# DCMMC/halo2-scaffold

Measured on NVIDIA B200. Metric: bn254_g1_msm_points_per_s, higher is better.
Workload: dtype u32 limbs (254-bit modular integers)

## Files before the change

halo2_scaffold_b200/csrc/ec.cuh:

```cuda
#pragma once
#include "field.cuh"

namespace h2b {

struct Affine {
    Fq x, y;
};
struct XYZZ {
    Fq x, y, zz, zzz;
};

__device__ __forceinline__ bool affine_is_identity(const Affine& p) { return fp_is_zero(p.x) && fp_is_zero(p.y); }
__device__ __forceinline__ bool xyzz_is_identity(const XYZZ& p) { return fp_is_zero(p.zz); }
__device__ __forceinline__ XYZZ xyzz_identity() {
    XYZZ r;
    r.x = fp_zero<FQ>(); r.y = fp_zero<FQ>(); r.zz = fp_zero<FQ>(); r.zzz = fp_zero<FQ>();
    return r;
}
__device__ __forceinline__ Affine affine_load(const void* p) {
    Affine a;
    a.x = fp_load<FQ>(p);
    a.y = fp_load<FQ>(reinterpret_cast<const uint4*>(p) + 2);
    return a;
}
// ... 65 lines not shown
    Affine q = q_in;
    if (neg) q.y = fp_neg(q.y);
    if (xyzz_is_identity(acc)) {
        acc.x = q.x; acc.y = q.y; acc.zz = fp_one<FQ>(); acc.zzz = fp_one<FQ>();
        return;
    }
    Fq u2 = fp_mul(q.x, acc.zz);
    Fq s2 = fp_mul(q.y, acc.zzz);
    Fq p = fp_sub(u2, acc.x);
    Fq r = fp_sub(s2, acc.y);
    if (fp_is_zero(p)) {
        if (fp_is_zero(r)) acc = xyzz_double_affine(q);
        else acc = xyzz_identity();
        return;
    }
    Fq pp = fp_sqr(p);
    Fq ppp = fp_mul(p, pp);
    Fq qq = fp_mul(acc.x, pp);
    Fq x3 = fp_sub(fp_sub(fp_sqr(r), ppp), fp_dbl(qq));
#ifdef H2B_MADD_MUL2
    Fq y3 = fp_mul2(r, fp_sub(qq, x3), fp_neg(acc.y), ppp);
#else
    Fq y3 = fp_sub(fp_mul(r, fp_sub(qq, x3)), fp_mul(acc.y, ppp));
#endif
    acc.x = x3;
    acc.y = y3;
    acc.zz = fp_mul(acc.zz, pp);
    acc.zzz = fp_mul(acc.zzz, ppp);
}

__device__ __forceinline__ void xyzz_add_affine_lazy(XYZZ& acc, const Affine& q_in, bool neg) {
    if (affine_is_identity(q_in)) return;
    Affine q = q_in;
    if (neg) q.y = fp_neg(q.y);
    if (xyzz_is_identity(acc)) {
        acc.x = q.x; acc.y = q.y; acc.zz = fp_one<FQ>(); acc.zzz = fp_one<FQ>();
        return;
    }
    Fq u2 = fp_mul_lazy(q.x, acc.zz);
    Fq s2 = fp_mul_lazy(q.y, acc.zzz);
    Fq p = fp_sub_lazy(u2, acc.x);
    Fq r = fp_sub_lazy(s2, acc.y);
    if (fp_is_zero_lazy(p)) {
        if (fp_is_zero_lazy(r)) acc = xyzz_double_affine(q);
        else acc = xyzz_identity();
        return;
    }
    Fq pp = fp_sqr_lazy(p);
    Fq ppp = fp_mul_lazy(p, pp);
    Fq qq = fp_mul_lazy(acc.x, pp);
    Fq yppp = fp_mul_lazy(acc.y, ppp);
    Fq x3 = fp_sub_lazy(fp_sub_lazy(fp_sqr_lazy(r), ppp), fp_add_lazy(qq, qq));
    Fq y3 = fp_sub_lazy(fp_mul_lazy(r, fp_sub_lazy(qq, x3)), yppp);
    acc.x = x3;
    acc.y = y3;
    acc.zz = fp_mul_lazy(acc.zz, pp);
    acc.zzz = fp_mul_lazy(acc.zzz, ppp);
}
__device__ __forceinline__ XYZZ xyzz_canon(const XYZZ& a) {
    XYZZ r;
    r.x = fp_canon(a.x); r.y = fp_canon(a.y); r.zz = fp_canon(a.zz); r.zzz = fp_canon(a.zzz);
    return r;
}

template <bool SHARED> __device__ __forceinline__ void xyzz_add_body(XYZZ& acc, const XYZZ& b);
static __device__ __noinline__ XYZZ xyzz_add_shared(XYZZ acc, XYZZ b) {
    xyzz_add_body<true>(acc, b);
    return acc;
}
template <bool SHARED = false>
__device__ __forceinline__ void xyzz_add(XYZZ& acc, const XYZZ& b) {
    if (SHARED) acc = xyzz_add_shared(acc, b);
    else xyzz_add_body<false>(acc, b);
}
template <bool SHARED>
__device__ __forceinline__ void xyzz_add_body(XYZZ& acc, const XYZZ& b) {
    if (xyzz_is_identity(b)) return;
    if (xyzz_is_identity(acc)) { acc = b; return; }
    Fq u1 = fq_m<SHARED>(acc.x, b.zz);
    Fq u2 = fq_m<SHARED>(b.x, acc.zz);
    Fq s1 = fq_m<SHARED>(acc.y, b.zzz);
    Fq s2 = fq_m<SHARED>(b.y, acc.zzz);
    Fq p = fp_sub(u2, u1);
    Fq r = fp_sub(s2, s1);
    if (fp_is_zero(p)) {
// ... 76 lines not shown
```

halo2_scaffold_b200/csrc/field.cuh:

```cuda
#pragma once
#include <cstdint>

#ifdef H2B_EMU
#include "cuda_emu.h"
#else
#include <cuda_runtime.h>
#define H2B_LAUNCH(kern, grid, block, smem, stream, ...) \
    (h2b::count_launch(), kern<<<(grid), (block), (smem), (stream)>>>(__VA_ARGS__))
#define H2B_DYN_SMEM(T, name)                                   \
    extern __shared__ __align__(16) unsigned char _h2b_dsm[];   \
    T* name = reinterpret_cast<T*>(_h2b_dsm)
#include "field_asm.inc"
#endif

namespace h2b {

extern unsigned long long g_launch_count;
inline void count_launch() { __atomic_fetch_add(&g_launch_count, 1ull, __ATOMIC_RELAXED); }

enum FieldId { FR = 0, FQ = 1 };

template <int F> struct FpParams;
template <> struct FpParams<FR> {
    __host__ __device__ static constexpr uint32_t P(int i) {
// ... 101 lines not shown
    Fp<F> r;
    if (F == FR) fr_sub_asm(r.l, a.l, b.l); else fq_sub_asm(r.l, a.l, b.l);
    return r;
}
template <int F> __device__ __forceinline__ Fp<F> fp_mul_lazy(const Fp<F>& a, const Fp<F>& b) {
    Fp<F> r;
    if (F == FR) fr_mul_lazy_asm(r.l, a.l, b.l); else fq_mul_lazy_asm(r.l, a.l, b.l);
    return r;
}
template <int F> __device__ __forceinline__ Fp<F> fp_sqr_lazy(const Fp<F>& a) {
#ifdef H2B_SQR_AS_MUL
    return fp_mul_lazy(a, a);
#else
    Fp<F> r;
    if (F == FR) fr_sqr_lazy_asm(r.l, a.l); else fq_sqr_lazy_asm(r.l, a.l);
    return r;
#endif
}
template <int F> __device__ __forceinline__ Fp<F> fp_add_lazy(const Fp<F>& a, const Fp<F>& b) {
    Fp<F> r;
    if (F == FR) fr_add_lazy_asm(r.l, a.l, b.l); else fq_add_lazy_asm(r.l, a.l, b.l);
    return r;
}
template <int F> __device__ __forceinline__ Fp<F> fp_sub_lazy(const Fp<F>& a, const Fp<F>& b) {
    Fp<F> r;
    if (F == FR) fr_sub_lazy_asm(r.l, a.l, b.l); else fq_sub_lazy_asm(r.l, a.l, b.l);
    return r;
}
template <int F> __device__ __forceinline__ Fp<F> fp_canon(const Fp<F>& a) {
    Fp<F> r;
    if (F == FR) fr_canon_asm(r.l, a.l); else fq_canon_asm(r.l, a.l);
    return r;
}
#else
template <int F> inline bool fp_geq_p(const uint32_t* t) {
    for (int i = 7; i >= 0; --i) {
        if (t[i] > FpParams<F>::P(i)) return true;
        if (t[i] < FpParams<F>::P(i)) return false;
    }
    return true;
}
template <int F> inline void fp_sub_p(uint32_t* t) {
    int64_t bw = 0;
    for (int i = 0; i < 8; ++i) {
        int64_t d = (int64_t)t[i] - FpParams<F>::P(i) + bw;
        t[i] = (uint32_t)d;
        bw = d >> 32;
    }
}
template <int F> inline void fp_mont_emu(const Fp<F>& a, const Fp<F>& b, uint32_t (&t)[10]) {
    for (int i = 0; i < 8; ++i) {
        uint64_t c = 0;
        for (int j = 0; j < 8; ++j) { c += (uint64_t)a.l[j] * b.l[i] + t[j]; t[j] = (uint32_t)c; c >>= 32; }
        c += t[8]; t[8] = (uint32_t)c; t[9] = (uint32_t)(c >> 32);
        uint32_t m = t[0] * FpParams<F>::INV;
        c = (uint64_t)m * FpParams<F>::P(0) + t[0]; c >>= 32;
        for (int j = 1; j < 8; ++j) { c += (uint64_t)m * FpParams<F>::P(j) + t[j]; t[j - 1] = (uint32_t)c; c >>= 32; }
        c += t[8]; t[7] = (uint32_t)c; t[8] = t[9] + (uint32_t)(c >> 32);
    }
}
template <int F> inline Fp<F> fp_mul(const Fp<F>& a, const Fp<F>& b) {
    uint32_t t[10] = {0};
    fp_mont_emu(a, b, t);
    Fp<F> r;
    if (t[8] || fp_geq_p<F>(t)) fp_sub_p<F>(t);
    for (int i = 0; i < 8; ++i) r.l[i] = t[i];
// ... 18 lines not shown
}
template <int F> inline void fp_2p(uint32_t (&q)[8]) {
    uint64_t c = 0;
    for (int i = 0; i < 8; ++i) { c += 2 * (uint64_t)FpParams<F>::P(i); q[i] = (uint32_t)c; c >>= 32; }
}
template <int F> inline Fp<F> fp_mul_lazy(const Fp<F>& a, const Fp<F>& b) {
    uint32_t t[10] = {0};
    fp_mont_emu(a, b, t);
    Fp<F> r; for (int i = 0; i < 8; ++i) r.l[i] = t[i];
    return r;
}
template <int F> inline Fp<F> fp_sqr_lazy(const Fp<F>& a) { return fp_mul_lazy(a, a); }
template <int F> inline Fp<F> fp_add_lazy(const Fp<F>& a, const Fp<F>& b) {
    uint32_t q[8], t[8], s[8]; fp_2p<F>(q);
    uint64_t c = 0; int64_t bw = 0;
    for (int i = 0; i < 8; ++i) { c += (uint64_t)a.l[i] + b.l[i]; t[i] = (uint32_t)c; c >>= 32; }
    for (int i = 0; i < 8; ++i) { int64_t d = (int64_t)t[i] - q[i] + bw; s[i] = (uint32_t)d; bw = d >> 32; }
    Fp<F> r; for (int i = 0; i < 8; ++i) r.l[i] = bw ? t[i] : s[i];
    return r;
}
template <int F> inline Fp<F> fp_sub_lazy(const Fp<F>& a, const Fp<F>& b) {
    uint32_t q[8], t[8]; fp_2p<F>(q);
    int64_t bw = 0;
    for (int i = 0; i < 8; ++i) { int64_t d = (int64_t)a.l[i] - b.l[i] + bw; t[i] = (uint32_t)d; bw = d >> 32; }
    if (bw) { uint64_t c = 0; for (int i = 0; i < 8; ++i) { c += (uint64_t)t[i] + q[i]; t[i] = (uint32_t)c; c >>= 32; } }
    Fp<F> r; for (int i = 0; i < 8; ++i) r.l[i] = t[i];
    return r;
}
template <int F> inline Fp<F> fp_canon(const Fp<F>& a) {
    Fp<F> r = a;
    if (fp_geq_p<F>(r.l)) fp_sub_p<F>(r.l);
    return r;
}
#endif

template <int F> __device__ __forceinline__ bool fp_is_zero_lazy(const Fp<F>& a) {
    uint32_t o = 0, d = 0;
#pragma unroll
    for (int i = 0; i < 8; ++i) { o |= a.l[i]; d |= a.l[i] ^ FpParams<F>::P(i); }
    return o == 0 || d == 0;
}

template <int F> __device__ __forceinline__ Fp<F> fp_neg(const Fp<F>& a) { return fp_sub(fp_zero<F>(), a); }
template <int F> __device__ __forceinline__ Fp<F> fp_dbl(const Fp<F>& a) { return fp_add(a, a); }
template <int F> __device__ __forceinline__ Fp<F> fp_from_mont(const Fp<F>& a) {
    Fp<F> o = fp_zero<F>();
    o.l[0] = 1;
    return fp_mul(a, o);
}
template <int F> __device__ __forceinline__ Fp<F> fp_to_mont(const Fp<F>& a) {
    Fp<F> r2;
#pragma unroll
    for (int i = 0; i < 8; ++i) r2.l[i] = FpParams<F>::R2(i);
    return fp_mul(a, r2);
}
template <int F> __device__ __noinline__ Fp<F> fp_inv(const Fp<F>& a) {
    Fp<F> r = fp_one<F>();
#pragma unroll
    for (int w = 7; w >= 0; --w) {
        uint32_t word = FpParams<F>::P(w);
        if (w == 0) word -= 2;
#pragma unroll 1
        for (int i = 31; i >= 0; --i) {
            r = fp_sqr(r);
            if ((word >> i) & 1) r = fp_mul(r, a);
        }
// ... 16 lines not shown
```

halo2_scaffold_b200/csrc/field_asm.inc:

```

__device__ __forceinline__ void fr_mul_asm(uint32_t (&r)[8], const uint32_t (&a)[8], const uint32_t (&b)[8]) {
    asm(
        "{\n\t"
        ".reg .u32 e0, e1, e2, e3, e4, e5, e6, e7, o0, o1, o2, o3, o4, o5, o6, o7, m, t0, t1, t2, t3, t4, t5, t6, t7, s0, s1, s2, s3, s4, s5, s6, s7, bw;\n\t"
        ".reg .pred pz;\n\t"
        "mul.lo.u32 o0, %9, %16;\n\t"
        "mul.hi.u32 o1, %9, %16;\n\t"
        "mul.lo.u32 o2, %11, %16;\n\t"
        "mul.hi.u32 o3, %11, %16;\n\t"
        "mul.lo.u32 o4, %13, %16;\n\t"
        "mul.hi.u32 o5, %13, %16;\n\t"
        "mul.lo.u32 o6, %15, %16;\n\t"
        "mul.hi.u32 o7, %15, %16;\n\t"
        "mul.lo.u32 e0, %8, %16;\n\t"
        "mul.hi.u32 e1, %8, %16;\n\t"
        "mul.lo.u32 e2, %10, %16;\n\t"
        "mul.hi.u32 e3, %10, %16;\n\t"
        "mul.lo.u32 e4, %12, %16;\n\t"
        "mul.hi.u32 e5, %12, %16;\n\t"
        "mul.lo.u32 e6, %14, %16;\n\t"
        "mul.hi.u32 e7, %14, %16;\n\t"
        "mul.lo.u32 m, e0, 0xefffffff;\n\t"
        "mad.lo.cc.u32 o0, 0x43e1f593, m, o0;\n\t"
        "madc.hi.cc.u32 o1, 0x43e1f593, m, o1;\n\t"
// ... 1222 lines not shown
        "sub.cc.u32 s0, t0, 0xf0000001;\n\t"
        "subc.cc.u32 s1, t1, 0x43e1f593;\n\t"
        "subc.cc.u32 s2, t2, 0x79b97091;\n\t"
        "subc.cc.u32 s3, t3, 0x2833e848;\n\t"
        "subc.cc.u32 s4, t4, 0x8181585d;\n\t"
        "subc.cc.u32 s5, t5, 0xb85045b6;\n\t"
        "subc.cc.u32 s6, t6, 0xe131a029;\n\t"
        "subc.cc.u32 s7, t7, 0x30644e72;\n\t"
        "subc.u32 bw, 0x00000000, 0x00000000;\n\t"
        "setp.ne.u32 pz, bw, 0;\n\t"
        "selp.u32 %0, t0, s0, pz;\n\t"
        "setp.ne.u32 pz, bw, 0;\n\t"
        "selp.u32 %1, t1, s1, pz;\n\t"
        "setp.ne.u32 pz, bw, 0;\n\t"
        "selp.u32 %2, t2, s2, pz;\n\t"
        "setp.ne.u32 pz, bw, 0;\n\t"
        "selp.u32 %3, t3, s3, pz;\n\t"
        "setp.ne.u32 pz, bw, 0;\n\t"
        "selp.u32 %4, t4, s4, pz;\n\t"
        "setp.ne.u32 pz, bw, 0;\n\t"
        "selp.u32 %5, t5, s5, pz;\n\t"
        "setp.ne.u32 pz, bw, 0;\n\t"
        "selp.u32 %6, t6, s6, pz;\n\t"
        "setp.ne.u32 pz, bw, 0;\n\t"
        "selp.u32 %7, t7, s7, pz;\n\t"
        "}\n\t"
        : "=r"(r[0]), "=r"(r[1]), "=r"(r[2]), "=r"(r[3]), "=r"(r[4]), "=r"(r[5]), "=r"(r[6]), "=r"(r[7])
        : "r"(a[0]), "r"(a[1]), "r"(a[2]), "r"(a[3]), "r"(a[4]), "r"(a[5]), "r"(a[6]), "r"(a[7]), "r"(b[0]), "r"(b[1]), "r"(b[2]), "r"(b[3]), "r"(b[4]), "r"(b[5]), "r"(b[6]), "r"(b[7]));
}

__device__ __forceinline__ void fr_sub_asm(uint32_t (&r)[8], const uint32_t (&a)[8], const uint32_t (&b)[8]) {
    asm(
        "{\n\t"
        ".reg .u32 t0, t1, t2, t3, t4, t5, t6, t7, q0, q1, q2, q3, q4, q5, q6, q7, bw;\n\t"
        ".reg .pred pz;\n\t"
        "sub.cc.u32 t0, %8, %16;\n\t"
        "subc.cc.u32 t1, %9, %17;\n\t"
        "subc.cc.u32 t2, %10, %18;\n\t"
        "subc.cc.u32 t3, %11, %19;\n\t"
        "subc.cc.u32 t4, %12, %20;\n\t"
        "subc.cc.u32 t5, %13, %21;\n\t"
        "subc.cc.u32 t6, %14, %22;\n\t"
        "subc.cc.u32 t7, %15, %23;\n\t"
        "subc.u32 bw, 0x00000000, 0x00000000;\n\t"
        "and.b32 q0, bw, 0xf0000001;\n\t"
        "and.b32 q1, bw, 0x43e1f593;\n\t"
        "and.b32 q2, bw, 0x79b97091;\n\t"
        "and.b32 q3, bw, 0x2833e848;\n\t"
        "and.b32 q4, bw, 0x8181585d;\n\t"
        "and.b32 q5, bw, 0xb85045b6;\n\t"
        "and.b32 q6, bw, 0xe131a029;\n\t"
        "and.b32 q7, bw, 0x30644e72;\n\t"
        "add.cc.u32 %0, t0, q0;\n\t"
        "addc.cc.u32 %1, t1, q1;\n\t"
        "addc.cc.u32 %2, t2, q2;\n\t"
        "addc.cc.u32 %3, t3, q3;\n\t"
        "addc.cc.u32 %4, t4, q4;\n\t"
        "addc.cc.u32 %5, t5, q5;\n\t"
        "addc.cc.u32 %6, t6, q6;\n\t"
        "addc.u32 %7, t7, q7;\n\t"
        "}\n\t"
        : "=r"(r[0]), "=r"(r[1]), "=r"(r[2]), "=r"(r[3]), "=r"(r[4]), "=r"(r[5]), "=r"(r[6]), "=r"(r[7])
        : "r"(a[0]), "r"(a[1]), "r"(a[2]), "r"(a[3]), "r"(a[4]), "r"(a[5]), "r"(a[6]), "r"(a[7]), "r"(b[0]), "r"(b[1]), "r"(b[2]), "r"(b[3]), "r"(b[4]), "r"(b[5]), "r"(b[6]), "r"(b[7]));
}

__device__ __forceinline__ void fq_mul_asm(uint32_t (&r)[8], const uint32_t (&a)[8], const uint32_t (&b)[8]) {
    asm(
// ... 1244 lines not shown
        "sub.cc.u32 s0, t0, 0xd87cfd47;\n\t"
        "subc.cc.u32 s1, t1, 0x3c208c16;\n\t"
        "subc.cc.u32 s2, t2, 0x6871ca8d;\n\t"
        "subc.cc.u32 s3, t3, 0x97816a91;\n\t"
        "subc.cc.u32 s4, t4, 0x8181585d;\n\t"
        "subc.cc.u32 s5, t5, 0xb85045b6;\n\t"
        "subc.cc.u32 s6, t6, 0xe131a029;\n\t"
        "subc.cc.u32 s7, t7, 0x30644e72;\n\t"
        "subc.u32 bw, 0x00000000, 0x00000000;\n\t"
        "setp.ne.u32 pz, bw, 0;\n\t"
        "selp.u32 %0, t0, s0, pz;\n\t"
        "setp.ne.u32 pz, bw, 0;\n\t"
        "selp.u32 %1, t1, s1, pz;\n\t"
        "setp.ne.u32 pz, bw, 0;\n\t"
        "selp.u32 %2, t2, s2, pz;\n\t"
        "setp.ne.u32 pz, bw, 0;\n\t"
        "selp.u32 %3, t3, s3, pz;\n\t"
        "setp.ne.u32 pz, bw, 0;\n\t"
        "selp.u32 %4, t4, s4, pz;\n\t"
        "setp.ne.u32 pz, bw, 0;\n\t"
        "selp.u32 %5, t5, s5, pz;\n\t"
        "setp.ne.u32 pz, bw, 0;\n\t"
        "selp.u32 %6, t6, s6, pz;\n\t"
        "setp.ne.u32 pz, bw, 0;\n\t"
        "selp.u32 %7, t7, s7, pz;\n\t"
        "}\n\t"
        : "=r"(r[0]), "=r"(r[1]), "=r"(r[2]), "=r"(r[3]), "=r"(r[4]), "=r"(r[5]), "=r"(r[6]), "=r"(r[7])
        : "r"(a[0]), "r"(a[1]), "r"(a[2]), "r"(a[3]), "r"(a[4]), "r"(a[5]), "r"(a[6]), "r"(a[7]), "r"(b[0]), "r"(b[1]), "r"(b[2]), "r"(b[3]), "r"(b[4]), "r"(b[5]), "r"(b[6]), "r"(b[7]));
}

__device__ __forceinline__ void fq_sub_asm(uint32_t (&r)[8], const uint32_t (&a)[8], const uint32_t (&b)[8]) {
    asm(
        "{\n\t"
        ".reg .u32 t0, t1, t2, t3, t4, t5, t6, t7, q0, q1, q2, q3, q4, q5, q6, q7, bw;\n\t"
        ".reg .pred pz;\n\t"
        "sub.cc.u32 t0, %8, %16;\n\t"
        "subc.cc.u32 t1, %9, %17;\n\t"
        "subc.cc.u32 t2, %10, %18;\n\t"
        "subc.cc.u32 t3, %11, %19;\n\t"
        "subc.cc.u32 t4, %12, %20;\n\t"
        "subc.cc.u32 t5, %13, %21;\n\t"
        "subc.cc.u32 t6, %14, %22;\n\t"
        "subc.cc.u32 t7, %15, %23;\n\t"
        "subc.u32 bw, 0x00000000, 0x00000000;\n\t"
        "and.b32 q0, bw, 0xd87cfd47;\n\t"
        "and.b32 q1, bw, 0x3c208c16;\n\t"
        "and.b32 q2, bw, 0x6871ca8d;\n\t"
        "and.b32 q3, bw, 0x97816a91;\n\t"
        "and.b32 q4, bw, 0x8181585d;\n\t"
        "and.b32 q5, bw, 0xb85045b6;\n\t"
        "and.b32 q6, bw, 0xe131a029;\n\t"
        "and.b32 q7, bw, 0x30644e72;\n\t"
        "add.cc.u32 %0, t0, q0;\n\t"
        "addc.cc.u32 %1, t1, q1;\n\t"
        "addc.cc.u32 %2, t2, q2;\n\t"
        "addc.cc.u32 %3, t3, q3;\n\t"
        "addc.cc.u32 %4, t4, q4;\n\t"
        "addc.cc.u32 %5, t5, q5;\n\t"
        "addc.cc.u32 %6, t6, q6;\n\t"
        "addc.u32 %7, t7, q7;\n\t"
        "}\n\t"
        : "=r"(r[0]), "=r"(r[1]), "=r"(r[2]), "=r"(r[3]), "=r"(r[4]), "=r"(r[5]), "=r"(r[6]), "=r"(r[7])
        : "r"(a[0]), "r"(a[1]), "r"(a[2]), "r"(a[3]), "r"(a[4]), "r"(a[5]), "r"(a[6]), "r"(a[7]), "r"(b[0]), "r"(b[1]), "r"(b[2]), "r"(b[3]), "r"(b[4]), "r"(b[5]), "r"(b[6]), "r"(b[7]));
}


__device__ __forceinline__ void fr_mul_lazy_asm(uint32_t (&r)[8], const uint32_t (&a)[8], const uint32_t (&b)[8]) {
// ... 660 lines not shown
        "sub.cc.u32 s0, t0, 0xe0000002;\n\t"
        "subc.cc.u32 s1, t1, 0x87c3eb27;\n\t"
        "subc.cc.u32 s2, t2, 0xf372e122;\n\t"
        "subc.cc.u32 s3, t3, 0x5067d090;\n\t"
        "subc.cc.u32 s4, t4, 0x0302b0ba;\n\t"
        "subc.cc.u32 s5, t5, 0x70a08b6d;\n\t"
        "subc.cc.u32 s6, t6, 0xc2634053;\n\t"
        "subc.cc.u32 s7, t7, 0x60c89ce5;\n\t"
        "subc.u32 bw, 0x00000000, 0x00000000;\n\t"
        "setp.ne.u32 pz, bw, 0;\n\t"
        "selp.u32 %0, t0, s0, pz;\n\t"
        "setp.ne.u32 pz, bw, 0;\n\t"
        "selp.u32 %1, t1, s1, pz;\n\t"
        "setp.ne.u32 pz, bw, 0;\n\t"
        "selp.u32 %2, t2, s2, pz;\n\t"
        "setp.ne.u32 pz, bw, 0;\n\t"
        "selp.u32 %3, t3, s3, pz;\n\t"
        "setp.ne.u32 pz, bw, 0;\n\t"
        "selp.u32 %4, t4, s4, pz;\n\t"
        "setp.ne.u32 pz, bw, 0;\n\t"
        "selp.u32 %5, t5, s5, pz;\n\t"
        "setp.ne.u32 pz, bw, 0;\n\t"
        "selp.u32 %6, t6, s6, pz;\n\t"
        "setp.ne.u32 pz, bw, 0;\n\t"
        "selp.u32 %7, t7, s7, pz;\n\t"
        "}\n\t"
        : "=r"(r[0]), "=r"(r[1]), "=r"(r[2]), "=r"(r[3]), "=r"(r[4]), "=r"(r[5]), "=r"(r[6]), "=r"(r[7])
        : "r"(a[0]), "r"(a[1]), "r"(a[2]), "r"(a[3]), "r"(a[4]), "r"(a[5]), "r"(a[6]), "r"(a[7]), "r"(b[0]), "r"(b[1]), "r"(b[2]), "r"(b[3]), "r"(b[4]), "r"(b[5]), "r"(b[6]), "r"(b[7]));
}

__device__ __forceinline__ void fr_sub_lazy_asm(uint32_t (&r)[8], const uint32_t (&a)[8], const uint32_t (&b)[8]) {
    asm(
        "{\n\t"
        ".reg .u32 t0, t1, t2, t3, t4, t5, t6, t7, q0, q1, q2, q3, q4, q5, q6, q7, bw;\n\t"
        ".reg .pred pz;\n\t"
        "sub.cc.u32 t0, %8, %16;\n\t"
        "subc.cc.u32 t1, %9, %17;\n\t"
        "subc.cc.u32 t2, %10, %18;\n\t"
        "subc.cc.u32 t3, %11, %19;\n\t"
        "subc.cc.u32 t4, %12, %20;\n\t"
        "subc.cc.u32 t5, %13, %21;\n\t"
        "subc.cc.u32 t6, %14, %22;\n\t"
        "subc.cc.u32 t7, %15, %23;\n\t"
        "subc.u32 bw, 0x00000000, 0x00000000;\n\t"
        "and.b32 q0, bw, 0xe0000002;\n\t"
        "and.b32 q1, bw, 0x87c3eb27;\n\t"
        "and.b32 q2, bw, 0xf372e122;\n\t"
        "and.b32 q3, bw, 0x5067d090;\n\t"
        "and.b32 q4, bw, 0x0302b0ba;\n\t"
        "and.b32 q5, bw, 0x70a08b6d;\n\t"
        "and.b32 q6, bw, 0xc2634053;\n\t"
        "and.b32 q7, bw, 0x60c89ce5;\n\t"
        "add.cc.u32 %0, t0, q0;\n\t"
        "addc.cc.u32 %1, t1, q1;\n\t"
        "addc.cc.u32 %2, t2, q2;\n\t"
        "addc.cc.u32 %3, t3, q3;\n\t"
        "addc.cc.u32 %4, t4, q4;\n\t"
        "addc.cc.u32 %5, t5, q5;\n\t"
        "addc.cc.u32 %6, t6, q6;\n\t"
        "addc.u32 %7, t7, q7;\n\t"
        "}\n\t"
        : "=r"(r[0]), "=r"(r[1]), "=r"(r[2]), "=r"(r[3]), "=r"(r[4]), "=r"(r[5]), "=r"(r[6]), "=r"(r[7])
        : "r"(a[0]), "r"(a[1]), "r"(a[2]), "r"(a[3]), "r"(a[4]), "r"(a[5]), "r"(a[6]), "r"(a[7]), "r"(b[0]), "r"(b[1]), "r"(b[2]), "r"(b[3]), "r"(b[4]), "r"(b[5]), "r"(b[6]), "r"(b[7]));
}

__device__ __forceinline__ void fr_canon_asm(uint32_t (&r)[8], const uint32_t (&a)[8]) {
    asm(
        "{\n\t"
        ".reg .u32 s0, s1, s2, s3, s4, s5, s6, s7, bw;\n\t"
        ".reg .pred pz;\n\t"
        "sub.cc.u32 s0, %8, 0xf0000001;\n\t"
        "subc.cc.u32 s1, %9, 0x43e1f593;\n\t"
        "subc.cc.u32 s2, %10, 0x79b97091;\n\t"
        "subc.cc.u32 s3, %11, 0x2833e848;\n\t"
        "subc.cc.u32 s4, %12, 0x8181585d;\n\t"
        "subc.cc.u32 s5, %13, 0xb85045b6;\n\t"
        "subc.cc.u32 s6, %14, 0xe131a029;\n\t"
        "subc.cc.u32 s7, %15, 0x30644e72;\n\t"
        "subc.u32 bw, 0x00000000, 0x00000000;\n\t"
        "setp.ne.u32 pz, bw, 0;\n\t"
        "selp.u32 %0, %8, s0, pz;\n\t"
        "setp.ne.u32 pz, bw, 0;\n\t"
        "selp.u32 %1, %9, s1, pz;\n\t"
        "setp.ne.u32 pz, bw, 0;\n\t"
        "selp.u32 %2, %10, s2, pz;\n\t"
        "setp.ne.u32 pz, bw, 0;\n\t"
        "selp.u32 %3, %11, s3, pz;\n\t"
        "setp.ne.u32 pz, bw, 0;\n\t"
        "selp.u32 %4, %12, s4, pz;\n\t"
        "setp.ne.u32 pz, bw, 0;\n\t"
        "selp.u32 %5, %13, s5, pz;\n\t"
        "setp.ne.u32 pz, bw, 0;\n\t"
        "selp.u32 %6, %14, s6, pz;\n\t"
        "setp.ne.u32 pz, bw, 0;\n\t"
        "selp.u32 %7, %15, s7, pz;\n\t"
        "}\n\t"
        : "=r"(r[0]), "=r"(r[1]), "=r"(r[2]), "=r"(r[3]), "=r"(r[4]), "=r"(r[5]), "=r"(r[6]), "=r"(r[7])
        : "r"(a[0]), "r"(a[1]), "r"(a[2]), "r"(a[3]), "r"(a[4]), "r"(a[5]), "r"(a[6]), "r"(a[7]));
}

__device__ __forceinline__ void fq_mul_lazy_asm(uint32_t (&r)[8], const uint32_t (&a)[8], const uint32_t (&b)[8]) {
    asm(
        "{\n\t"
        ".reg .u32 e0, e1, e2, e3, e4, e5, e6, e7, o0, o1, o2, o3, o4, o5, o6, o7, m;\n\t"
        ".reg .pred pz;\n\t"
        "mul.lo.u32 o0, %9, %16;\n\t"
        "mul.hi.u32 o1, %9, %16;\n\t"
        "mul.lo.u32 o2, %11, %16;\n\t"
        "mul.hi.u32 o3, %11, %16;\n\t"
        "mul.lo.u32 o4, %13, %16;\n\t"
        "mul.hi.u32 o5, %13, %16;\n\t"
        "mul.lo.u32 o6, %15, %16;\n\t"
        "mul.hi.u32 o7, %15, %16;\n\t"
        "mul.lo.u32 e0, %8, %16;\n\t"
        "mul.hi.u32 e1, %8, %16;\n\t"
        "mul.lo.u32 e2, %10, %16;\n\t"
        "mul.hi.u32 e3, %10, %16;\n\t"
        "mul.lo.u32 e4, %12, %16;\n\t"
        "mul.hi.u32 e5, %12, %16;\n\t"
        "mul.lo.u32 e6, %14, %16;\n\t"
        "mul.hi.u32 e7, %14, %16;\n\t"
        "mul.lo.u32 m, e0, 0xe4866389;\n\t"
        "mad.lo.cc.u32 o0, 0x3c208c16, m, o0;\n\t"
        "madc.hi.cc.u32 o1, 0x3c208c16, m, o1;\n\t"
        "madc.lo.cc.u32 o2, 0x97816a91, m, o2;\n\t"
        "madc.hi.cc.u32 o3, 0x97816a91, m, o3;\n\t"
        "madc.lo.cc.u32 o4, 0xb85045b6, m, o4;\n\t"
        "madc.hi.cc.u32 o5, 0xb85045b6, m, o5;\n\t"
        "madc.lo.cc.u32 o6, 0x30644e72, m, o6;\n\t"
        "madc.hi.cc.u32 o7, 0x30644e72, m, o7;\n\t"
        "mad.lo.cc.u32 e0, 0xd87cfd47, m, e0;\n\t"
// ... 630 lines not shown
        "sub.cc.u32 s0, t0, 0xb0f9fa8e;\n\t"
        "subc.cc.u32 s1, t1, 0x7841182d;\n\t"
        "subc.cc.u32 s2, t2, 0xd0e3951a;\n\t"
        "subc.cc.u32 s3, t3, 0x2f02d522;\n\t"
        "subc.cc.u32 s4, t4, 0x0302b0bb;\n\t"
        "subc.cc.u32 s5, t5, 0x70a08b6d;\n\t"
        "subc.cc.u32 s6, t6, 0xc2634053;\n\t"
        "subc.cc.u32 s7, t7, 0x60c89ce5;\n\t"
        "subc.u32 bw, 0x00000000, 0x00000000;\n\t"
        "setp.ne.u32 pz, bw, 0;\n\t"
        "selp.u32 %0, t0, s0, pz;\n\t"
        "setp.ne.u32 pz, bw, 0;\n\t"
        "selp.u32 %1, t1, s1, pz;\n\t"
        "setp.ne.u32 pz, bw, 0;\n\t"
        "selp.u32 %2, t2, s2, pz;\n\t"
        "setp.ne.u32 pz, bw, 0;\n\t"
        "selp.u32 %3, t3, s3, pz;\n\t"
        "setp.ne.u32 pz, bw, 0;\n\t"
        "selp.u32 %4, t4, s4, pz;\n\t"
        "setp.ne.u32 pz, bw, 0;\n\t"
        "selp.u32 %5, t5, s5, pz;\n\t"
        "setp.ne.u32 pz, bw, 0;\n\t"
        "selp.u32 %6, t6, s6, pz;\n\t"
        "setp.ne.u32 pz, bw, 0;\n\t"
        "selp.u32 %7, t7, s7, pz;\n\t"
        "}\n\t"
        : "=r"(r[0]), "=r"(r[1]), "=r"(r[2]), "=r"(r[3]), "=r"(r[4]), "=r"(r[5]), "=r"(r[6]), "=r"(r[7])
        : "r"(a[0]), "r"(a[1]), "r"(a[2]), "r"(a[3]), "r"(a[4]), "r"(a[5]), "r"(a[6]), "r"(a[7]), "r"(b[0]), "r"(b[1]), "r"(b[2]), "r"(b[3]), "r"(b[4]), "r"(b[5]), "r"(b[6]), "r"(b[7]));
}

__device__ __forceinline__ void fq_sub_lazy_asm(uint32_t (&r)[8], const uint32_t (&a)[8], const uint32_t (&b)[8]) {
    asm(
        "{\n\t"
        ".reg .u32 t0, t1, t2, t3, t4, t5, t6, t7, q0, q1, q2, q3, q4, q5, q6, q7, bw;\n\t"
        ".reg .pred pz;\n\t"
        "sub.cc.u32 t0, %8, %16;\n\t"
        "subc.cc.u32 t1, %9, %17;\n\t"
        "subc.cc.u32 t2, %10, %18;\n\t"
        "subc.cc.u32 t3, %11, %19;\n\t"
        "subc.cc.u32 t4, %12, %20;\n\t"
        "subc.cc.u32 t5, %13, %21;\n\t"
        "subc.cc.u32 t6, %14, %22;\n\t"
        "subc.cc.u32 t7, %15, %23;\n\t"
        "subc.u32 bw, 0x00000000, 0x00000000;\n\t"
        "and.b32 q0, bw, 0xb0f9fa8e;\n\t"
        "and.b32 q1, bw, 0x7841182d;\n\t"
        "and.b32 q2, bw, 0xd0e3951a;\n\t"
        "and.b32 q3, bw, 0x2f02d522;\n\t"
        "and.b32 q4, bw, 0x0302b0bb;\n\t"
        "and.b32 q5, bw, 0x70a08b6d;\n\t"
        "and.b32 q6, bw, 0xc2634053;\n\t"
        "and.b32 q7, bw, 0x60c89ce5;\n\t"
        "add.cc.u32 %0, t0, q0;\n\t"
        "addc.cc.u32 %1, t1, q1;\n\t"
        "addc.cc.u32 %2, t2, q2;\n\t"
        "addc.cc.u32 %3, t3, q3;\n\t"
        "addc.cc.u32 %4, t4, q4;\n\t"
        "addc.cc.u32 %5, t5, q5;\n\t"
        "addc.cc.u32 %6, t6, q6;\n\t"
        "addc.u32 %7, t7, q7;\n\t"
        "}\n\t"
        : "=r"(r[0]), "=r"(r[1]), "=r"(r[2]), "=r"(r[3]), "=r"(r[4]), "=r"(r[5]), "=r"(r[6]), "=r"(r[7])
        : "r"(a[0]), "r"(a[1]), "r"(a[2]), "r"(a[3]), "r"(a[4]), "r"(a[5]), "r"(a[6]), "r"(a[7]), "r"(b[0]), "r"(b[1]), "r"(b[2]), "r"(b[3]), "r"(b[4]), "r"(b[5]), "r"(b[6]), "r"(b[7]));
}

__device__ __forceinline__ void fq_canon_asm(uint32_t (&r)[8], const uint32_t (&a)[8]) {
    asm(
        "{\n\t"
        ".reg .u32 s0, s1, s2, s3, s4, s5, s6, s7, bw;\n\t"
        ".reg .pred pz;\n\t"
        "sub.cc.u32 s0, %8, 0xd87cfd47;\n\t"
        "subc.cc.u32 s1, %9, 0x3c208c16;\n\t"
        "subc.cc.u32 s2, %10, 0x6871ca8d;\n\t"
        "subc.cc.u32 s3, %11, 0x97816a91;\n\t"
        "subc.cc.u32 s4, %12, 0x8181585d;\n\t"
        "subc.cc.u32 s5, %13, 0xb85045b6;\n\t"
        "subc.cc.u32 s6, %14, 0xe131a029;\n\t"
        "subc.cc.u32 s7, %15, 0x30644e72;\n\t"
        "subc.u32 bw, 0x00000000, 0x00000000;\n\t"
        "setp.ne.u32 pz, bw, 0;\n\t"
        "selp.u32 %0, %8, s0, pz;\n\t"
        "setp.ne.u32 pz, bw, 0;\n\t"
        "selp.u32 %1, %9, s1, pz;\n\t"
        "setp.ne.u32 pz, bw, 0;\n\t"
        "selp.u32 %2, %10, s2, pz;\n\t"
        "setp.ne.u32 pz, bw, 0;\n\t"
        "selp.u32 %3, %11, s3, pz;\n\t"
        "setp.ne.u32 pz, bw, 0;\n\t"
        "selp.u32 %4, %12, s4, pz;\n\t"
        "setp.ne.u32 pz, bw, 0;\n\t"
        "selp.u32 %5, %13, s5, pz;\n\t"
        "setp.ne.u32 pz, bw, 0;\n\t"
        "selp.u32 %6, %14, s6, pz;\n\t"
        "setp.ne.u32 pz, bw, 0;\n\t"
        "selp.u32 %7, %15, s7, pz;\n\t"
        "}\n\t"
        : "=r"(r[0]), "=r"(r[1]), "=r"(r[2]), "=r"(r[3]), "=r"(r[4]), "=r"(r[5]), "=r"(r[6]), "=r"(r[7])
        : "r"(a[0]), "r"(a[1]), "r"(a[2]), "r"(a[3]), "r"(a[4]), "r"(a[5]), "r"(a[6]), "r"(a[7]));
}
```

halo2_scaffold_b200/csrc/msm.cu:

```cuda
#include "common.h"
#include "ec.cuh"

namespace h2b {

static const uint32_t SIGN_BIT = 0x80000000u;

#if defined(H2B_EMU) || defined(H2B_NO_STREAMING_STORES)
#define H2B_STORE_STREAMING(ptr, val) (*(ptr) = (val))
#else
#define H2B_STORE_STREAMING(ptr, val) __stcs((ptr), (val))
#endif

struct MsmPlan {
    uint32_t n;
    uint32_t c;
    uint32_t W;
    uint32_t m;
    uint32_t Nb;
    uint32_t B;
    uint32_t stride;
    uint32_t row0;
    uint32_t G;
    uint32_t add_into;
    uint32_t top_bins;
// ... 504 lines not shown
        if (live) {
            for (uint32_t w = 1; w < lower; ++w) {
                uint32_t e = digits[(size_t)w * pl.n + i];
                if (e != 0) {
                    uint32_t d = e & ~SIGN_BIT;
                    uint32_t pos = atomicAdd(&cursor[set * pl.Nb + d - 1], 1u);
                    H2B_STORE_STREAMING(&sorted[pos], row | (e & SIGN_BIT));
                }
                if (++set == pl.m) { set = 0; row += pl.stride; }
            }
        }
        if (pl.top_bins) {
            for (uint32_t b = threadIdx.x; b < pl.top_bins; b += blockDim.x) top_cnt[b] = 0;
            __syncthreads();
            uint32_t e = live ? digits[(size_t)(pl.W - 1) * pl.n + i] : 0u;
            uint32_t d = e & ~SIGN_BIT, rank = 0;
            if (d) rank = atomicAdd(&top_cnt[d], 1u);
            __syncthreads();
            for (uint32_t b = 1 + threadIdx.x; b < pl.top_bins; b += blockDim.x)
                if (top_cnt[b]) top_cnt[b] = atomicAdd(&cursor[top_set * pl.Nb + b - 1], top_cnt[b]);
            __syncthreads();
            if (d) sorted[top_cnt[d] + rank] = (pl.row0 + i + ((pl.W - 1) / pl.m) * pl.stride) | (e & SIGN_BIT);
            __syncthreads();
        }
    }
}

static const uint32_t SLICE_MIN = 16;
__device__ __forceinline__ uint32_t slice_len(uint32_t total, uint32_t G) {
    uint32_t S = (total + G - 1) / G;
    return S < SLICE_MIN ? SLICE_MIN : S;
}

__global__ void __launch_bounds__(256) msm_accumulate_kernel(MsmPlan pl, const uint4* __restrict__ tables, const uint32_t* __restrict__ offsets,
                                                           const uint32_t* __restrict__ sorted, uint32_t* __restrict__ ctrl,
                                                           uint32_t* __restrict__ split_list, uint4* __restrict__ bucket_acc,
                                                           uint4* __restrict__ head_partial) {
    const uint32_t t = blockIdx.x * blockDim.x + threadIdx.x;
    if (t >= pl.G) return;
    const uint32_t total = offsets[pl.B];
    const uint32_t S = slice_len(total, pl.G);
    if ((uint64_t)t * S >= total) return;
    const uint32_t start = t * S;
    const uint32_t end = (total - start > S) ? start + S : total;
    uint32_t lo = 0, hi = pl.B;
    while (hi - lo > 1) {
        uint32_t mid = (lo + hi) >> 1;
        if (offsets[mid] <= start) lo = mid; else hi = mid;
    }
    uint32_t b = lo;
    uint32_t next = offsets[b + 1];
    bool head = offsets[b] < start;

    XYZZ acc = xyzz_identity();
    uint32_t e = sorted[start];
    Affine p = affine_load(tables + 4 * (size_t)(e & ~SIGN_BIT));
    for (uint32_t j = start; j < end; ++j) {
        uint32_t e_next = 0;
        Affine p_next = p;
        if (j + 1 < end) {
            e_next = sorted[j + 1];
            p_next = affine_load(tables + 4 * (size_t)(e_next & ~SIGN_BIT));
        }
        if (j == next) {
            if (head) xyzz_store(head_partial + 8 * (size_t)t, xyzz_canon(acc));
            else xyzz_store(bucket_acc + 8 * (size_t)b, xyzz_canon(acc));
            head = false;
            acc = xyzz_identity();
            do { ++b; next = offsets[b + 1]; } while (next <= j);
        }
        xyzz_add_affine_lazy(acc, p, (e & SIGN_BIT) != 0);
        e = e_next;
        p = p_next;
    }
    if (head) {
        xyzz_store(head_partial + 8 * (size_t)t, xyzz_canon(acc));
    } else {
        xyzz_store(bucket_acc + 8 * (size_t)b, xyzz_canon(acc));
        if (next > end) split_list[atomicAdd(&ctrl[0], 1u)] = b;
    }
}

static const uint32_t COMBINE_HEAVY = 24;
static const uint32_t COMBINE_CHUNK = 1024;
static const uint32_t COMBINE_THREADS = 256;

struct HeavyDesc { uint32_t bucket, chunk0, nchunks, pad; };

__global__ void __launch_bounds__(128) msm_combine_light_kernel(MsmPlan pl, const uint32_t* __restrict__ offsets, uint32_t* __restrict__ ctrl,
                                                              const uint32_t* __restrict__ split_list, HeavyDesc* __restrict__ heavy,
                                                              uint2* __restrict__ chunk_desc, const uint4* __restrict__ head_partial,
                                                              uint4* __restrict__ bucket_acc) {
    const uint32_t idx = blockIdx.x * blockDim.x + threadIdx.x;
    if (idx >= ctrl[0]) return;
    const uint32_t S = slice_len(offsets[pl.B], pl.G);
    const uint32_t b = split_list[idx];
// ... 785 lines not shown
```

Baseline: 427.6 million.

## Make mixed-add branchless and add min-blocks launch bound to accumulate kernel

The lazy mixed addition now negates the affine y with a predicated conditional-negate and folds the accumulator-identity check into the rare p==0 branch. The Fq lazy subtraction uses a predicated add of the modulus instead of mask-and-add, x3 uses two subtractions instead of an add, and the prefetch in the accumulate loop is made unconditional by clamping the index. The kernel also gets a minimum of 2 blocks per SM in its launch bounds, capping registers. Together these aim to cut warp divergence, instruction count and register pressure, but the register cap risks spills.

```diff
diff --git a/halo2_scaffold_b200/csrc/ec.cuh b/halo2_scaffold_b200/csrc/ec.cuh
--- a/halo2_scaffold_b200/csrc/ec.cuh
+++ b/halo2_scaffold_b200/csrc/ec.cuh
@@ -121,17 +121,14 @@
 __device__ __forceinline__ void xyzz_add_affine_lazy(XYZZ& acc, const Affine& q_in, bool neg) {
     if (affine_is_identity(q_in)) return;
     Affine q = q_in;
-    if (neg) q.y = fp_neg(q.y);
-    if (xyzz_is_identity(acc)) {
-        acc.x = q.x; acc.y = q.y; acc.zz = fp_one<FQ>(); acc.zzz = fp_one<FQ>();
-        return;
-    }
+    q.y = fp_cneg(q.y, neg);
     Fq u2 = fp_mul_lazy(q.x, acc.zz);
     Fq s2 = fp_mul_lazy(q.y, acc.zzz);
     Fq p = fp_sub_lazy(u2, acc.x);
     Fq r = fp_sub_lazy(s2, acc.y);
     if (fp_is_zero_lazy(p)) {
-        if (fp_is_zero_lazy(r)) acc = xyzz_double_affine(q);
+        if (xyzz_is_identity(acc)) { acc.x = q.x; acc.y = q.y; acc.zz = fp_one<FQ>(); acc.zzz = fp_one<FQ>(); }
+        else if (fp_is_zero_lazy(r)) acc = xyzz_double_affine(q);
         else acc = xyzz_identity();
         return;
     }
@@ -139,7 +136,7 @@
     Fq ppp = fp_mul_lazy(p, pp);
     Fq qq = fp_mul_lazy(acc.x, pp);
     Fq yppp = fp_mul_lazy(acc.y, ppp);
-    Fq x3 = fp_sub_lazy(fp_sub_lazy(fp_sqr_lazy(r), ppp), fp_add_lazy(qq, qq));
+    Fq x3 = fp_sub_lazy(fp_sub_lazy(fp_sub_lazy(fp_sqr_lazy(r), ppp), qq), qq);
     Fq y3 = fp_sub_lazy(fp_mul_lazy(r, fp_sub_lazy(qq, x3)), yppp);
     acc.x = x3;
     acc.y = y3;
diff --git a/halo2_scaffold_b200/csrc/field.cuh b/halo2_scaffold_b200/csrc/field.cuh
--- a/halo2_scaffold_b200/csrc/field.cuh
+++ b/halo2_scaffold_b200/csrc/field.cuh
@@ -157,6 +157,11 @@
     if (F == FR) fr_canon_asm(r.l, a.l); else fq_canon_asm(r.l, a.l);
     return r;
 }
+template <int F> __device__ __forceinline__ Fp<F> fp_cneg(const Fp<F>& a, bool neg) {
+    Fp<F> r;
+    if (F == FR) fr_cneg_asm(r.l, a.l, (uint32_t)neg); else fq_cneg_asm(r.l, a.l, (uint32_t)neg);
+    return r;
+}
 #else
 template <int F> inline bool fp_geq_p(const uint32_t* t) {
     for (int i = 7; i >= 0; --i) {
@@ -241,6 +246,13 @@
     if (fp_geq_p<F>(r.l)) fp_sub_p<F>(r.l);
     return r;
 }
+template <int F> inline Fp<F> fp_cneg(const Fp<F>& a, bool neg) {
+    if (!neg) return a;
+    Fp<F> r;
+    int64_t bw = 0;
+    for (int i = 0; i < 8; ++i) { int64_t d = (int64_t)FpParams<F>::P(i) - a.l[i] + bw; r.l[i] = (uint32_t)d; bw = d >> 32; }
+    return r;
+}
 #endif
 
 template <int F> __device__ __forceinline__ bool fp_is_zero_lazy(const Fp<F>& a) {
diff --git a/halo2_scaffold_b200/csrc/field_asm.inc b/halo2_scaffold_b200/csrc/field_asm.inc
--- a/halo2_scaffold_b200/csrc/field_asm.inc
+++ b/halo2_scaffold_b200/csrc/field_asm.inc
@@ -1278,7 +1278,7 @@
 __device__ __forceinline__ void fr_sub_asm(uint32_t (&r)[8], const uint32_t (&a)[8], const uint32_t (&b)[8]) {
     asm(
         "{\n\t"
-        ".reg .u32 t0, t1, t2, t3, t4, t5, t6, t7, q0, q1, q2, q3, q4, q5, q6, q7, bw;\n\t"
+        ".reg .u32 t0, t1, t2, t3, t4, t5, t6, t7, bw, q0, q1, q2, q3, q4, q5, q6, q7;\n\t"
         ".reg .pred pz;\n\t"
         "sub.cc.u32 t0, %8, %16;\n\t"
         "subc.cc.u32 t1, %9, %17;\n\t"
@@ -2589,7 +2589,7 @@
 __device__ __forceinline__ void fq_sub_asm(uint32_t (&r)[8], const uint32_t (&a)[8], const uint32_t (&b)[8]) {
     asm(
         "{\n\t"
-        ".reg .u32 t0, t1, t2, t3, t4, t5, t6, t7, q0, q1, q2, q3, q4, q5, q6, q7, bw;\n\t"
+        ".reg .u32 t0, t1, t2, t3, t4, t5, t6, t7, bw, q0, q1, q2, q3, q4, q5, q6, q7;\n\t"
         ".reg .pred pz;\n\t"
         "sub.cc.u32 t0, %8, %16;\n\t"
         "subc.cc.u32 t1, %9, %17;\n\t"
@@ -3316,7 +3316,7 @@
 __device__ __forceinline__ void fr_sub_lazy_asm(uint32_t (&r)[8], const uint32_t (&a)[8], const uint32_t (&b)[8]) {
     asm(
         "{\n\t"
-        ".reg .u32 t0, t1, t2, t3, t4, t5, t6, t7, q0, q1, q2, q3, q4, q5, q6, q7, bw;\n\t"
+        ".reg .u32 t0, t1, t2, t3, t4, t5, t6, t7, bw, q0, q1, q2, q3, q4, q5, q6, q7;\n\t"
         ".reg .pred pz;\n\t"
         "sub.cc.u32 t0, %8, %16;\n\t"
         "subc.cc.u32 t1, %9, %17;\n\t"
@@ -3381,6 +3381,32 @@
         "}\n\t"
         : "=r"(r[0]), "=r"(r[1]), "=r"(r[2]), "=r"(r[3]), "=r"(r[4]), "=r"(r[5]), "=r"(r[6]), "=r"(r[7])
         : "r"(a[0]), "r"(a[1]), "r"(a[2]), "r"(a[3]), "r"(a[4]), "r"(a[5]), "r"(a[6]), "r"(a[7]));
+}
+
+__device__ __forceinline__ void fr_cneg_asm(uint32_t (&r)[8], const uint32_t (&a)[8], uint32_t f) {
+    asm(
+        "{\n\t"
+        ".reg .pred pz;\n\t"
+        "mov.u32 %0, %8;\n\t"
+        "mov.u32 %1, %9;\n\t"
+        "mov.u32 %2, %10;\n\t"
+        "mov.u32 %3, %11;\n\t"
+        "mov.u32 %4, %12;\n\t"
+        "mov.u32 %5, %13;\n\t"
+        "mov.u32 %6, %14;\n\t"
+        "mov.u32 %7, %15;\n\t"
+        "setp.ne.u32 pz, %16, 0;\n\t"
+        "@pz sub.cc.u32 %0, 0xf0000001, %0;\n\t"
+        "@pz subc.cc.u32 %1, 0x43e1f593, %1;\n\t"
+        "@pz subc.cc.u32 %2, 0x79b97091, %2;\n\t"
+        "@pz subc.cc.u32 %3, 0x2833e848, %3;\n\t"
+        "@pz subc.cc.u32 %4, 0x8181585d, %4;\n\t"
+        "@pz subc.cc.u32 %5, 0xb85045b6, %5;\n\t"
+        "@pz subc.cc.u32 %6, 0xe131a029, %6;\n\t"
+        "@pz subc.u32 %7, 0x30644e72, %7;\n\t"
+        "}\n\t"
+        : "=r"(r[0]), "=r"(r[1]), "=r"(r[2]), "=r"(r[3]), "=r"(r[4]), "=r"(r[5]), "=r"(r[6]), "=r"(r[7])
+        : "r"(a[0]), "r"(a[1]), "r"(a[2]), "r"(a[3]), "r"(a[4]), "r"(a[5]), "r"(a[6]), "r"(a[7]), "r"(f));
 }
 
 __device__ __forceinline__ void fq_mul_lazy_asm(uint32_t (&r)[8], const uint32_t (&a)[8], const uint32_t (&b)[8]) {
@@ -4077,7 +4103,7 @@
 __device__ __forceinline__ void fq_sub_lazy_asm(uint32_t (&r)[8], const uint32_t (&a)[8], const uint32_t (&b)[8]) {
     asm(
         "{\n\t"
-        ".reg .u32 t0, t1, t2, t3, t4, t5, t6, t7, q0, q1, q2, q3, q4, q5, q6, q7, bw;\n\t"
+        ".reg .u32 t0, t1, t2, t3, t4, t5, t6, t7, bw;\n\t"
         ".reg .pred pz;\n\t"
         "sub.cc.u32 t0, %8, %16;\n\t"
         "subc.cc.u32 t1, %9, %17;\n\t"
@@ -4088,22 +4114,23 @@
         "subc.cc.u32 t6, %14, %22;\n\t"
         "subc.cc.u32 t7, %15, %23;\n\t"
         "subc.u32 bw, 0x00000000, 0x00000000;\n\t"
-        "and.b32 q0, bw, 0xb0f9fa8e;\n\t"
-        "and.b32 q1, bw, 0x7841182d;\n\t"
-        "and.b32 q2, bw, 0xd0e3951a;\n\t"
-        "and.b32 q3, bw, 0x2f02d522;\n\t"
-        "and.b32 q4, bw, 0x0302b0bb;\n\t"
-        "and.b32 q5, bw, 0x70a08b6d;\n\t"
-        "and.b32 q6, bw, 0xc2634053;\n\t"
-        "and.b32 q7, bw, 0x60c89ce5;\n\t"
-        "add.cc.u32 %0, t0, q0;\n\t"
-        "addc.cc.u32 %1, t1, q1;\n\t"
-        "addc.cc.u32 %2, t2, q2;\n\t"
-        "addc.cc.u32 %3, t3, q3;\n\t"
-        "addc.cc.u32 %4, t4, q4;\n\t"
-        "addc.cc.u32 %5, t5, q5;\n\t"
-        "addc.cc.u32 %6, t6, q6;\n\t"
-        "addc.u32 %7, t7, q7;\n\t"
+        "setp.ne.u32 pz, bw, 0;\n\t"
+        "@pz add.cc.u32 t0, t0, 0xb0f9fa8e;\n\t"
+        "@pz addc.cc.u32 t1, t1, 0x7841182d;\n\t"
+        "@pz addc.cc.u32 t2, t2, 0xd0e3951a;\n\t"
+        "@pz addc.cc.u32 t3, t3, 0x2f02d522;\n\t"
+        "@pz addc.cc.u32 t4, t4, 0x0302b0bb;\n\t"
+        "@pz addc.cc.u32 t5, t5, 0x70a08b6d;\n\t"
+        "@pz addc.cc.u32 t6, t6, 0xc2634053;\n\t"
+        "@pz addc.u32 t7, t7, 0x60c89ce5;\n\t"
+        "mov.u32 %0, t0;\n\t"
+        "mov.u32 %1, t1;\n\t"
+        "mov.u32 %2, t2;\n\t"
+        "mov.u32 %3, t3;\n\t"
+        "mov.u32 %4, t4;\n\t"
+        "mov.u32 %5, t5;\n\t"
+        "mov.u32 %6, t6;\n\t"
+        "mov.u32 %7, t7;\n\t"
         "}\n\t"
         : "=r"(r[0]), "=r"(r[1]), "=r"(r[2]), "=r"(r[3]), "=r"(r[4]), "=r"(r[5]), "=r"(r[6]), "=r"(r[7])
         : "r"(a[0]), "r"(a[1]), "r"(a[2]), "r"(a[3]), "r"(a[4]), "r"(a[5]), "r"(a[6]), "r"(a[7]), "r"(b[0]), "r"(b[1]), "r"(b[2]), "r"(b[3]), "r"(b[4]), "r"(b[5]), "r"(b[6]), "r"(b[7]));
@@ -4143,3 +4170,29 @@
         : "=r"(r[0]), "=r"(r[1]), "=r"(r[2]), "=r"(r[3]), "=r"(r[4]), "=r"(r[5]), "=r"(r[6]), "=r"(r[7])
         : "r"(a[0]), "r"(a[1]), "r"(a[2]), "r"(a[3]), "r"(a[4]), "r"(a[5]), "r"(a[6]), "r"(a[7]));
 }
+
+__device__ __forceinline__ void fq_cneg_asm(uint32_t (&r)[8], const uint32_t (&a)[8], uint32_t f) {
+    asm(
+        "{\n\t"
+        ".reg .pred pz;\n\t"
+        "mov.u32 %0, %8;\n\t"
+        "mov.u32 %1, %9;\n\t"
+        "mov.u32 %2, %10;\n\t"
+        "mov.u32 %3, %11;\n\t"
+        "mov.u32 %4, %12;\n\t"
+        "mov.u32 %5, %13;\n\t"
+        "mov.u32 %6, %14;\n\t"
+        "mov.u32 %7, %15;\n\t"
+        "setp.ne.u32 pz, %16, 0;\n\t"
+        "@pz sub.cc.u32 %0, 0xd87cfd47, %0;\n\t"
+        "@pz subc.cc.u32 %1, 0x3c208c16, %1;\n\t"
+        "@pz subc.cc.u32 %2, 0x6871ca8d, %2;\n\t"
+        "@pz subc.cc.u32 %3, 0x97816a91, %3;\n\t"
+        "@pz subc.cc.u32 %4, 0x8181585d, %4;\n\t"
+        "@pz subc.cc.u32 %5, 0xb85045b6, %5;\n\t"
+        "@pz subc.cc.u32 %6, 0xe131a029, %6;\n\t"
+        "@pz subc.u32 %7, 0x30644e72, %7;\n\t"
+        "}\n\t"
+        : "=r"(r[0]), "=r"(r[1]), "=r"(r[2]), "=r"(r[3]), "=r"(r[4]), "=r"(r[5]), "=r"(r[6]), "=r"(r[7])
+        : "r"(a[0]), "r"(a[1]), "r"(a[2]), "r"(a[3]), "r"(a[4]), "r"(a[5]), "r"(a[6]), "r"(a[7]), "r"(f));
+}
diff --git a/halo2_scaffold_b200/csrc/msm.cu b/halo2_scaffold_b200/csrc/msm.cu
--- a/halo2_scaffold_b200/csrc/msm.cu
+++ b/halo2_scaffold_b200/csrc/msm.cu
@@ -560,7 +560,7 @@
     return S < SLICE_MIN ? SLICE_MIN : S;
 }
 
-__global__ void __launch_bounds__(256) msm_accumulate_kernel(MsmPlan pl, const uint4* __restrict__ tables, const uint32_t* __restrict__ offsets,
+__global__ void __launch_bounds__(256, 2) msm_accumulate_kernel(MsmPlan pl, const uint4* __restrict__ tables, const uint32_t* __restrict__ offsets,
                                                            const uint32_t* __restrict__ sorted, uint32_t* __restrict__ ctrl,
                                                            uint32_t* __restrict__ split_list, uint4* __restrict__ bucket_acc,
                                                            uint4* __restrict__ head_partial) {
@@ -584,12 +584,8 @@
     uint32_t e = sorted[start];
     Affine p = affine_load(tables + 4 * (size_t)(e & ~SIGN_BIT));
     for (uint32_t j = start; j < end; ++j) {
-        uint32_t e_next = 0;
-        Affine p_next = p;
-        if (j + 1 < end) {
-            e_next = sorted[j + 1];
-            p_next = affine_load(tables + 4 * (size_t)(e_next & ~SIGN_BIT));
-        }
+        const uint32_t e_next = sorted[j + 1 < end ? j + 1 : j];
+        const Affine p_next = affine_load(tables + 4 * (size_t)(e_next & ~SIGN_BIT));
         if (j == next) {
             if (head) xyzz_store(head_partial + 8 * (size_t)t, xyzz_canon(acc));
             else xyzz_store(bucket_acc + 8 * (size_t)b, xyzz_canon(acc));
```

Result: faster. 436.8 million (median of 6 runs) (+2.2%).
